# JustinMLu/legged_gym_custom

Measured on AMD Instinct MI355X. Metric: env-steps/sec (whole node), Go2 4096 envs, 1/2/4/8 MI355X, higher is better.
Workload: dtype f32; 1 GPU; go2, rsl_rl PPO/ROA iteration (24 env steps + 5x4 minibatch update); num_envs_per_gpu=4096, num_steps_per_env=24, global_envs=4096, parallelism=env-sharded dp1

## Files before the change

include/lgx.h:

```cpp
#ifndef LGX_H
#define LGX_H

#include <stdint.h>

#ifdef __cplusplus
extern "C" {
#endif

#define LGX_ABI_VERSION 13

#define LGX_MAX_DOF 12
#define LGX_MAX_LINKS 16
#define LGX_MAX_BODIES 24
#define LGX_MAX_FEET 4
#define LGX_MAX_PROPRIO 240
#define LGX_MAX_HEIGHT_POINTS 192
#define LGX_MAX_REWARDS 40
#define LGX_MAX_CANDIDATES 64
#define LGX_MAX_CONTACTS 16
#define LGX_MAX_PENALISED 24
#define LGX_MAX_TERMINATION 8
#define LGX_EVAL_METRICS 8
#define LGX_EVAL_CELL_COLS 12
#define LGX_MAX_ACTION_HISTORY 4
// ... 226 lines not shown
int64_t lgx_sizeof_task_params(void);
int64_t lgx_sizeof_buffers(void);

int lgx_create(const lgx_model* model, const lgx_task_params* params, int32_t device, lgx_env** out);
int lgx_bind(lgx_env* env, const lgx_buffers* buffers);
int lgx_step(lgx_env* env, uint64_t seed, uint64_t step_counter, void* hip_stream);
int lgx_step_dev(lgx_env* env, uint64_t seed, const uint64_t* d_step_counter, void* hip_stream);
int lgx_post_physics(lgx_env* env, uint64_t seed, uint64_t step_counter, void* hip_stream);
int lgx_physics(lgx_env* env, void* hip_stream);
int lgx_reset_envs(lgx_env* env, const uint8_t* env_mask, uint64_t seed, uint64_t reset_call, void* hip_stream);
int lgx_episode_extras(lgx_env* env, float* means, float* level_mean, uint8_t* time_outs, uint64_t* step_dev,
                       void* hip_stream);
int lgx_command_curriculum(lgx_env* env, uint64_t seed, uint64_t step_counter, const uint64_t* d_step_counter,
                           const double* global_sum_count, void* hip_stream);
int lgx_set_envs_per_wave(lgx_env* env, int32_t envs_per_wave);

typedef struct lgx_eval_buffers {
  float* acc;
  uint8_t* status;
  double* cells;
  uint32_t* overflow;
  int32_t cell_rows, cell_cols;
  const int32_t* cell_ids;
  float* push_rec;
  float settle_tol;
  double* push_cells;
  const int32_t* cmd_switch_step;
  float* cmd_rec;
  double* cmd_cells;
  float yaw_tol;
// ... 52 lines not shown
```

legged_gym_custom_amd/_abi.py:

```python
import ctypes as C

ABI_VERSION = 13
MAX_DOF = 12
MAX_LINKS = 16
MAX_BODIES = 24
MAX_FEET = 4
MAX_PROPRIO = 240
MAX_HEIGHT_POINTS = 192
MAX_REWARDS = 40
MAX_CANDIDATES = 64
MAX_CONTACTS = 16
MAX_PENALISED = 24
MAX_TERMINATION = 8
EVAL_METRICS = 8
EVAL_CELL_COLS = 12
MAX_ACTION_HISTORY = 4
EVAL_PUSH_REC = 4
EVAL_PUSH_COLS = 5
CMD_SEGMENTS = 4
EVAL_CMD_REC = 8
EVAL_CMD_COLS = 9
TRACE_COLS = 76
GAIT_FOOT_COLS = 16
GAIT_BODY_COLS = 12
# ... 167 lines not shown

u64, cint = C.c_uint64, C.c_int
SIGNATURES = {
    "lgx_abi_version": (i32, ()),
    **{name: (C.c_int64, ()) for name in SIZEOF},
    "lgx_create": (cint, (P, P, i32, C.POINTER(P))),
    "lgx_bind": (cint, (P, P)),
    "lgx_step": (cint, (P, u64, u64, P)),
    "lgx_step_dev": (cint, (P, u64, P, P)),
    "lgx_post_physics": (cint, (P, u64, u64, P)),
    "lgx_physics": (cint, (P, P)),
    "lgx_reset_envs": (cint, (P, P, u64, u64, P)),
    "lgx_episode_extras": (cint, (P, P, P, P, P, P)),
    "lgx_command_curriculum": (cint, (P, u64, u64, P, P, P)),
    "lgx_set_envs_per_wave": (cint, (P, i32)),
    "lgx_eval_begin": (cint, (P, P, P)),
    "lgx_eval_accumulate": (cint, (P, P, P)),
    "lgx_eval_reduce": (cint, (P, P, P)),
    "lgx_trace_begin": (cint, (P, P, P)),
    "lgx_trace_record": (cint, (P, P, P)),
    "lgx_trace_gather": (cint, (P, P, P, i32, P, P, P)),
    "lgx_gait_begin": (cint, (P, P, P)),
    "lgx_gait_record": (cint, (P, P, P)),
    "lgx_gait_reduce": (cint, (P, P, P)),
    "lgx_joint_begin": (cint, (P, P, P)),
    "lgx_joint_record": (cint, (P, P, P)),
    "lgx_joint_reduce": (cint, (P, P, P)),
    "lgx_last_error": (C.c_char_p, (P,)),
    "lgx_destroy": (None, (P,)),
}
# ... 12 lines not shown
```

legged_gym_custom_amd/_native.py:

```python
import ctypes as C
import os

from . import _abi, _cbind

LIB_PATH = os.environ.get("LGX_LIB") or os.path.join(os.path.dirname(os.path.abspath(__file__)), "lib", "liblgx.so")
_lib = None


class LgxError(RuntimeError):
    pass


def lib():
    global _lib
    if _lib is None:
        _lib = _cbind.load(LIB_PATH, "liblgx", _abi.SIGNATURES, _abi.STRUCTS, ("lgx_abi_version", _abi.ABI_VERSION),
                           _abi.SIZEOF, LgxError)
    return _lib


EXPORTED = list(_abi.SIGNATURES)


class NativeEnv:
# ... 20 lines not shown
            t = tensors.get(name)
            if t is None:
                setattr(self.buffers, name, None)
                continue
            if not t.is_contiguous():
                raise LgxError(f"buffer {name} must be contiguous")
            if t.device.type != self._dev_type:
                where = "host memory (device -1)" if self._dev_type == "cpu" else "the HIP device"
                raise LgxError(f"buffer {name} must live in {where} (got {t.device})")
            setattr(self.buffers, name, t.data_ptr())
            self._keep[name] = t
        self._check(self._L.lgx_bind(self.handle, C.byref(self.buffers)), "lgx_bind")

    def set_envs_per_wave(self, n):
        self._check(self._L.lgx_set_envs_per_wave(self.handle, int(n)), "lgx_set_envs_per_wave")

    def step(self, seed, step_counter, stream):
        self._check(self._L.lgx_step(self.handle, seed, step_counter, C.c_void_p(stream)), "lgx_step")

    def step_dev(self, seed, step_counter_tensor, stream):
        self._check(self._L.lgx_step_dev(self.handle, seed, C.c_void_p(step_counter_tensor.data_ptr()),
                                         C.c_void_p(stream)), "lgx_step_dev")

    def post_physics(self, seed, step_counter, stream):
        self._check(self._L.lgx_post_physics(self.handle, seed, step_counter, C.c_void_p(stream)), "lgx_post_physics")

    def reset_envs(self, mask, seed, call, stream):
        self._keep["_mask"] = mask
        self._check(self._L.lgx_reset_envs(self.handle, C.c_void_p(mask.data_ptr()), seed, call, C.c_void_p(stream)),
                    "lgx_reset_envs")
# ... 145 lines not shown
```

legged_gym_custom_amd/csrc/lgx_env.hip:

```cpp
#include <hip/hip_runtime.h>
#include "lgx_knobs.h"
#include <math.h>
#include <stddef.h>
#include <stdint.h>

#include "../../include/lgx.h"
#include "lgx_device.h"
#include "lgx_env_common.h"
#include "lgx_host.h"

namespace lgx {

constexpr int ASQ = 24;
constexpr int AMAX = 33;
constexpr int RW = 9;
constexpr int A_FLOATS = ASQ * ASQ > AMAX * (AMAX + 1) / 2 ? ASQ * ASQ : AMAX * (AMAX + 1) / 2;
constexpr int J9_FLOATS = MAXR * RW > A_FLOATS ? MAXR * RW : A_FLOATS;
constexpr int ROWS_FLOATS = MAXR * RW + J9_FLOATS;
extern __shared__ float lgx_dyn[];
struct DynTemps {
  float Fw[NL][3], Nw[NL][3];
  float Dl[4][6];
  float tot[16];
  float Sp[21];
};
static_assert(sizeof(DynTemps) <= ROWS_FLOATS * sizeof(float), "dynamics temporaries fit the arena");
LGX_DEV DynTemps& dtmp(float* A) { return *reinterpret_cast<DynTemps*>(A); }
LGX_DEV float* stg_U(float* A) { return A; }
LGX_DEV float* stg_cur(float* A, const lgx_task_params* Pm) { return A + 4 * rng_blocks(Pm); }
constexpr int HIST_LDS_MAX = 640;
__host__ __device__ inline bool hist_in_lds(const lgx_task_params* Pm) {
  return Pm->history_len * Pm->num_proprio <= HIST_LDS_MAX || Pm->num_proprio < 64;
}
LGX_DEV float* stg_hist(float* A, const lgx_task_params* Pm) { return stg_cur(A, Pm) + Pm->num_proprio; }
LGX_DEV float* stg_heights(float* A, const lgx_task_params* Pm) {
  return stg_hist(A, Pm) + (hist_in_lds(Pm) ? Pm->history_len * Pm->num_proprio : 0);
}
__host__ __device__ inline int64_t arena_floats(const lgx_task_params& p) {
  const int64_t post = 4 * (9 + (p.num_proprio + 3) / 4) + p.num_proprio +
                       (hist_in_lds(&p) ? (int64_t)p.history_len * p.num_proprio : 0) + p.num_height_points;
  return post > ROWS_FLOATS ? post : ROWS_FLOATS;
}

struct Sh {
  Scratch x;
  float root[13], cmd[4], fat[4], lch[4];
  int lc[4];
  float rterm[64];
  float jsum[16];
  long long ep_prev;
  int lc_prev[LGX_MAX_FEET];
  float lch_prev[LGX_MAX_FEET], fat_prev[LGX_MAX_FEET], jump_prev;
  float la_prev[NJ], lt_prev[NJ];
  float es[LGX_MAX_REWARDS + 4];
  float fric;
  long long ep;
  int reset, tout;
  int blew;
  float qb[4], pb[3], vo[3], wb[3];
// ... 27 lines not shown
  } while (0)
#else
#define PH(k) \
  do {        \
  } while (0)
#endif

#pragma clang fp contract(fast)

template <class T>
LGX_DEV const T* opaque(const T* p) {
  __asm__ volatile("" : "+s"(p));
  return p;
}

LGX_DEV int env_of_block(int b, int n) {
  const int q = n >> 3, r = n & 7, x = b & 7, j = b >> 3;
  return x * q + min(x, r) + j;
}

#ifndef LGX_ROW_PRIO
#define LGX_ROW_PRIO 9
#endif
#ifndef LGX_SLOT_PRIO
#define LGX_SLOT_PRIO 0
#endif

LGX_DEV int wave_slot() { return __builtin_amdgcn_s_getreg(4 | (3 << 11)) & 15; }
LGX_DEV void set_prio(int p) {
  if (p >= 3) __builtin_amdgcn_s_setprio(3);
// ... 171 lines not shown
    const float on = lane <= NJ ? 1.f : 0.f;
    const float rd[16] = {m, m * r.x, m * r.y, m * r.z,
                          Iw[0] + m * (rr - r.x * r.x), Iw[1] + m * (rr - r.y * r.y), Iw[2] + m * (rr - r.z * r.z),
                          Iw[3] - m * r.x * r.y, Iw[4] - m * r.x * r.z, Iw[5] - m * r.y * r.z,
                          F.x, F.y, F.z, Nt.x, Nt.y, Nt.z};
#pragma unroll
    for (int q = 0; q < 16; ++q) {
      float x = rd[q] * on;
      x += dpp_shr_t<0x111>(x);
      x += dpp_shr_t<0x112>(x);
      x += dpp_shr_t<0x114>(x);
      x += dpp_shr_t<0x118>(x);
      if (lane == 15) dtmp(A).tot[q] = x;
    }
  }
  __syncthreads();
}

struct DynOut {
  float hb[6];
  float hj;
  float xj[6];
  float dinv[3];
};

LGX_DEV void dynamics(Sh& s, float* A, int lane, DynOut& o) {
  const f3 p0 = ld3(s.P[0]);
  const float* tot = dtmp(A).tot;
  const int j = lane < NJ ? lane : NJ - 1, l = j / 3, a = j % 3;
  if (lane < NJ) {
    const int kj = 1 + j;
// ... 19 lines not shown
    const int q = lane - 8, lq = q / 6, e = q % 6;
    const int j1 = e < 3 ? e : (e == 5 ? 1 : 0);
    const int j2 = e < 3 ? e : (e == 3 ? 1 : 2);
    const int k1 = 1 + 3 * lq + j1, k2 = 1 + 3 * lq + j2;
    const f3 a1 = ld3(s.Ax[k1]), a2 = ld3(s.Ax[k2]), p1 = ld3(s.P[k1]), p2 = ld3(s.P[k2]);
    float acc = 0.f;
#pragma unroll
    for (int i = 0; i < 3; ++i) {
      if (i < j2) continue;
      const int k = 1 + 3 * lq + i;
      const f3 c = ld3(s.C[k]);
      acc += s.m[k] * dot(cross(a1, c - p1), cross(a2, c - p2)) + dot(a1, symv(s.I[k], a2));
    }
    dtmp(A).Dl[lq][e] = acc;
  }
  __syncthreads();
  float Di[6];
  sym3_inv(dtmp(A).Dl[l], Di);
#pragma unroll
  for (int c = 0; c < 3; ++c) o.dinv[c] = sym3(Di, a, c);
  if (lane < NJ && a == 0) {
#pragma unroll
    for (int q = 0; q < 6; ++q) s.Dinv[l][q] = Di[q];
  }
  float bj[6];
  {
    const float* B0 = s.Bc[3 * l];
    const float* B1 = s.Bc[3 * l + 1];
    const float* B2 = s.Bc[3 * l + 2];
#pragma unroll
    for (int r = 0; r < 6; ++r) {
      const float b0 = B0[r], b1 = B1[r], b2 = B2[r];
      o.xj[r] = o.dinv[0] * b0 + o.dinv[1] * b1 + o.dinv[2] * b2;
      bj[r] = a == 0 ? b0 : (a == 1 ? b1 : b2);
    }
  }
  if (lane < NJ) {
#pragma unroll
    for (int r = 0; r < 6; ++r) s.X[j][r] = o.xj[r];
  }
  __syncthreads();
  if (lane < 21) {
    const int q = lane;
    const int r = (q >= 1) + (q >= 3) + (q >= 6) + (q >= 10) + (q >= 15), c = q - r * (r + 1) / 2;
    float acc = 0.f;
#pragma unroll
    for (int jj = 0; jj < NJ; ++jj) acc += s.X[jj][r] * s.Bc[jj][c];
    dtmp(A).Sp[q] = acc;
  }
  __syncthreads();
  const float Mt = tot[0], Hx = tot[1], Hy = tot[2], Hz = tot[3];
  const float Ab[21] = {Mt, 0.f, Mt, 0.f, 0.f, Mt, 0.f, -Hz, Hy, tot[4], Hz, 0.f, -Hx, tot[7], tot[5],
                        -Hy, Hx, 0.f, tot[8], tot[9], tot[6]};
  float L[21];
#pragma unroll
  for (int q = 0; q < 21; ++q) L[q] = Ab[q] - dtmp(A).Sp[q];
  float inv[6];
#pragma unroll
  for (int c = 0; c < 6; ++c) {
    float d = L[pk(c, c)];
#pragma unroll
    for (int k = 0; k < c; ++k) d -= L[pk(c, k)] * L[pk(c, k)];
    const float lcc = sqrtf(fmaxf(d, 1e-12f));
    inv[c] = 1.0f / lcc;
#pragma unroll
// ... 75 lines not shown
  const int total_max = gmax<WL>(total);
  int* const T_end = reinterpret_cast<int*>(A);
  int* const T_ci = T_end + 64;
  int* const T_cj = T_end + 128;
  int* const T_i0 = T_end + 192;
  int* const T_j0 = T_end + 256;
  int* const T_w = T_end + 320;
  float* const T_p = A + 384;
  float* const R_ = A + 576;
  T_end[lane] = endp; T_ci[lane] = ci; T_cj[lane] = cj; T_i0[lane] = i0; T_j0[lane] = j0; T_w[lane] = w;
  T_p[lane] = p.x; T_p[64 + lane] = p.y; T_p[128 + lane] = p.z;
  float best = 3.0e38f, zs = -3.0e38f;
  f3 q = mk(0.f, 0.f, -3.0e38f), fn = mk(0.f, 0.f, 1.f);
  const int mystart = endp - cnt;
  for (int base = 0; base < total_max; base += WL) {
    __syncthreads();
    const int t = base + lane;
    float td2 = 3.0e38f, tz = -3.0e38f;
    f3 tq = mk(0.f, 0.f, -3.0e38f), tfn = mk(0.f, 0.f, 1.f);
    if (t < total) {
      int lo = 0, hi = WL - 1;
      while (lo < hi) {
        const int mid = (lo + hi) >> 1;
        if (T_end[mid] > t) hi = mid; else lo = mid + 1;
      }
      const int c = lo;
      const int k = t - (c ? T_end[c - 1] : 0);
      const int wc = T_w[c];
      const int i = T_i0[c] + k / wc, j = T_j0[c] + k % wc;
      const int cci = T_ci[c], ccj = T_cj[c];
      const f3 pc = mk(T_p[c], T_p[64 + c], T_p[128 + c]);
// ... 4 lines not shown
#pragma unroll
      for (int tri = 0; tri < 2; ++tri) {
        const f3 a = v00, b = tri == 0 ? v11 : v10, cc = tri == 0 ? v01 : v11;
        const f3 cpt = closest_on_triangle(pc, a, b, cc);
        const f3 dd = pc - cpt;
        const float d2 = dot(dd, dd);
        if (d2 < td2) { td2 = d2; tq = cpt; tfn = cross(b - a, cc - a); }
        float z;
        if (height_in_triangle(pc, a, b, cc, z)) tz = fmaxf(tz, z);
      }
    }
    R_[lane] = td2;
    R_[64 + lane] = tq.x; R_[128 + lane] = tq.y; R_[192 + lane] = tq.z;
    R_[256 + lane] = tfn.x; R_[320 + lane] = tfn.y; R_[384 + lane] = tfn.z;
    R_[448 + lane] = tz;
    __syncthreads();
    if (cnt > 0) {
      const int a0 = max(mystart, base) - base, a1 = min(endp, base + WL) - base;
      for (int sl = a0; sl < a1; ++sl) {
        const float d2 = R_[sl];
        if (d2 < best) {
          best = d2;
          q = mk(R_[64 + sl], R_[128 + sl], R_[192 + sl]);
          fn = mk(R_[256 + sl], R_[320 + sl], R_[384 + sl]);
        }
        zs = fmaxf(zs, R_[448 + sl]);
      }
    }
  }
  __syncthreads();
  TerrainHit h;
  if (best >= 3.0e38f) {
    h.depth = -3.0e38f;
    h.n = mk(0.f, 0.f, 1.f);
    return h;
  }
  const float dist = sqrtf(best);
  const bool below = p.z < zs;
  h.depth = below ? r + dist : r - dist;
  if (dist > 1e-6f) {
    h.n = (p - q) * ((below ? -1.0f : 1.0f) / dist);
  } else {
    h.n = fn * rsqrtf(fmaxf(dot(fn, fn), 1e-30f));
  }
  return h;
// ... 83 lines not shown
  }
  return a;
}

LGX_DEV float motor_strength(const lgx_task_params* Pm, const lgx_buffers& B, int e, int j) {
  return B.motor_strength ? B.motor_strength[(size_t)e * Pm->num_dof + j] : 1.0f;
}

LGX_DEV void sea_torques_lanes(Sh& s, float* A, const lgx_task_params* Pm_, const lgx_buffers& B, int e, int lane,
                               int sub) {
  const size_t NT = (size_t)Pm_->num_envs * Pm_->num_dof;
  const int u = lane & 7;
  {
    const float* src = &Pm_->sea_in_scale[0];
    for (int i = lane; i < SEA_WN; i += 64) A[i] = src[i];
    __syncthreads();
  }
#pragma unroll 1
  for (int pass = 0; pass < 2; ++pass) {
    const lgx_task_params* Pm = opaque(Pm_);
    int wb = 0;
    __asm__ volatile("" : "+s"(wb));
    const SeaW W{A + wb};
    const int j = pass * 8 + (lane >> 3);
    const bool on = j < NJ;
    const int jj = on ? j : NJ - 1;
    const size_t r = (size_t)e * Pm->num_dof + jj;
    float h0 = B.sea_hidden[r * 8 + u], c0 = B.sea_cell[r * 8 + u];
    float h1 = B.sea_hidden[(NT + r) * 8 + u], c1 = B.sea_cell[(NT + r) * 8 + u];
    const float in0 = (sea_action(s, Pm, B, e, jj, sub) * Pm->action_scale + Pm->default_dof_pos[jj]) - s.th[jj];
    const float x[2] = {in0 * Pm->sea_in_scale[0], s.thd[jj] * Pm->sea_in_scale[1]};
// ... 57 lines not shown
      g[2] = Di[4] * jlr[0] + Di[5] * jlr[1] + Di[2] * jlr[2];
    }
    float* zg = ZG + lane * RW;
    float arr = jlr[0] * g[0] + jlr[1] * g[1] + jlr[2] * g[2];
#pragma unroll
    for (int q = 0; q < 6; ++q) {
      const float* Si = s.Sinv[q];
      const float zq = Si[0] * yr[0] + Si[1] * yr[1] + Si[2] * yr[2] + Si[3] * yr[3] + Si[4] * yr[4] + Si[5] * yr[5];
      zg[q] = zq;
      arr += yr[q] * zq;
    }
    zg[6] = g[0]; zg[7] = g[1]; zg[8] = g[2];
    s.Arr[lane] = arr;
    s.lam[lane] = 0.f;
  }
  __syncthreads();
  PH(6);
  const int NRm = gmax<WL>(nrows);
  const bool tri = nrows > ASQ, stored = nrows <= AMAX;
  if (stored && row_lane) {
#pragma unroll 4
    for (int q = 0; q < NRm; ++q) {
      if (q < nrows) {
        const float* zg = ZG + q * RW;
        const float v = yr[0] * zg[0] + yr[1] * zg[1] + yr[2] * zg[2] + yr[3] * zg[3] + yr[4] * zg[4] + yr[5] * zg[5];
        const float vl = jlr[0] * zg[6] + jlr[1] * zg[7] + jlr[2] * zg[8];
        const float a = v + (s.rleg[q] == lr ? vl : 0.f);
        if (!tri) Am[q * nrows + lane] = a;
        else if (q >= lane) Am[q * (q + 1) / 2 + lane] = a;
      }
    }
  }
  __syncthreads();
  PH(7);
  {
    float w = w0, lam = 0.f;
    const float mu = s.mu;
    auto wave_shl1 = [](float v) {
      return __int_as_float(__builtin_amdgcn_update_dpp(0, __float_as_int(v), 0x130, 0xf, 0xf, false));
    };
    auto wave_shr1 = [](float v) {
      return __int_as_float(__builtin_amdgcn_update_dpp(0, __float_as_int(v), 0x138, 0xf, 0xf, false));
    };
    const float tg = row_lane ? s.tgt[lane] : 0.f;
    const float ia = row_lane ? 1.0f / s.Arr[lane] : 0.f;
    const int rlast = max(nrows - 3, 0);
    const int lc = max(min(lane, nrows - 1), 0);
    const int tl = lc * (lc + 1) / 2;
// ... 55 lines not shown
          const float d1 = gbcast<WL>(dl, ra_ + 1, rb_ + 1), d2 = gbcast<WL>(dl, ra_ + 2, rb_ + 2);
          lam = sel((unsigned)(lane - r - 1) < 2u && on, lam, lt);
          w += a1 * d1 + a2 * d2;
        }
      }
    };
    if constexpr (WL == 64) {
      if (!stored) sweeps(arow_otf);
      else if (tri) sweeps(arow_tri);
      else sweeps(arow_sq);
    } else {
      sweeps(arow_mix);
    }
    if (row_lane) s.lam[lane] = lam;
  }
  __syncthreads();
  PH(8);
}

template <bool TERRAIN, bool ACTNET, int WL>
LGX_DEV void substep(Sh& s, float* A, Sh* S0, float* A0, int astride, const lgx_model* M_,
                     const lgx_task_params* Pm_, const lgx_buffers& B, int lane_, int e, int sub, bool last) {
  const lgx_model* M = opaque(M_);
  const lgx_task_params* Pm = opaque(Pm_);
  const int lane = opaque_lane(lane_);
  const float dt = Pm->sim_dt;
  {
#pragma clang fp contract(off)
    if (ACTNET) {
      sea_torques_lanes(s, A, Pm, B, e, lane, sub);
    } else if (lane < NJ) {
// ... 14 lines not shown
      if (B.motor_strength) t = motor_strength(Pm, B, e, j) * t;
      s.tau[j] = fminf(fmaxf(t, -Pm->torque_limits[j]), Pm->torque_limits[j]);
    }
  }
  PH(1);
  kinematics<true>(s, A, M, Pm, lane);
  PH(2);
  DynOut dy;
  dynamics(s, A, lane, dy);
  const int jl_ = lane < NJ ? lane : NJ - 1, leg_ = jl_ / 3, pos_ = jl_ % 3;
  const float fj = lane < NJ ? s.tau[lane] - dy.hj : 0.f;
  if (lane < NJ) s.up[lane] = fj;
  float vb[6];
#pragma unroll
  for (int r = 0; r < 6; ++r) vb[r] = -dy.hb[r] - grow_sum16<WL>(dy.xj[r] * fj);
  __syncthreads();
  PH(3);
  {
    float zb[6];
#pragma unroll
    for (int r = 0; r < 6; ++r) {
      const float* Si = s.Sinv[r];
      zb[r] = Si[0] * vb[0] + Si[1] * vb[1] + Si[2] * vb[2] + Si[3] * vb[3] + Si[4] * vb[4] + Si[5] * vb[5];
    }
    if (lane < 6) {
      const float* Si = s.Sinv[lane];
      const float zl = Si[0] * vb[0] + Si[1] * vb[1] + Si[2] * vb[2] + Si[3] * vb[3] + Si[4] * vb[4] + Si[5] * vb[5];
      const float u0 = lane < 3 ? s.vo[lane] : s.wb[lane - 3];
      s.us[lane] = u0 + dt * zl;
    }
    if (lane < NJ) {
// ... 116 lines not shown
  const int nrows = nlim + 3 * ncon;
  const int nrw = gmax<WL>(nrows);
#if LGX_ROW_PRIO > 0
  {
    const int rp = nrw > LGX_ROW_PRIO * 3 ? 3 : nrw > LGX_ROW_PRIO * 2 ? 2 : nrw > LGX_ROW_PRIO ? 1 : 0;
    set_prio(LGX_SLOT_PRIO ? max(rp, min(wave_slot(), 3)) : rp);
  }
#endif
  if (lane == 0) { s.nrows = nrows; s.nlim = nlim; s.ncon = ncon; }
#ifdef LGX_PHASE_CLOCK
  if (lane == 0) {
    s.phacc[16] = max(s.phacc[16], (uint32_t)nrows);
    s.phacc[17] += nrows > AMAX ? 1u : 0u;
  }
#endif
  __syncthreads();
  PH(5);
  if constexpr (WL == 64) {
    solve_rows<64>(s, A, Pm, lane, nrows, nlim, ncon);
  } else if (nrw <= WL) {
    solve_rows<WL>(s, A, Pm, lane, nrows, nlim, ncon);
  } else {
    const int wl = (int)__lane_id();
#pragma unroll 1
    for (int g = 0; g < 64 / WL; ++g) {
      Sh& sg = S0[g];
      const int nr = gval<WL>(nrows, g), nli = gval<WL>(nlim, g), nco = gval<WL>(ncon, g);
      solve_rows<64>(sg, A0 + (size_t)g * astride, Pm, wl, nr, nli, nco);
    }
  }
  {
// ... 12 lines not shown
    }
    if (lane < 6) {
      float zl = 0.f;
#pragma unroll
      for (int q = 0; q < 6; ++q) zl = lane == q ? Z[q] : zl;
      s.up[lane] = s.us[lane] + zl;
    }
    if (lane < NJ) {
      const float* Xj = s.X[lane];
      float v = s.us[6 + lane] + G;
#pragma unroll
      for (int q = 0; q < 6; ++q) v -= Xj[q] * Z[q];
      s.up[6 + lane] = v;
    }
  }
  __syncthreads();
  PH(9);
  if (last && lane < LGX_MAX_BODIES) {
    float f[3] = {0.f, 0.f, 0.f};
    const int ncm = gmax<WL>(ncon);
    for (int c = 0; c < ncm; ++c) {
      if (c >= ncon || s.cbody[c] != lane) continue;
      const int r = nlim + 3 * c;
      if constexpr (!TERRAIN) {
        f[2] += s.lam[r]; f[0] += s.lam[r + 1]; f[1] += s.lam[r + 2];
      } else {
        f3 t1, t2;
        const f3 n = ld3(s.cn[c]);
        contact_tangents(n, t1, t2);
        const f3 fc = n * s.lam[r] + t1 * s.lam[r + 1] + t2 * s.lam[r + 2];
        f[0] += fc.x; f[1] += fc.y; f[2] += fc.z;
// ... 18 lines not shown
    float qn[4];
    qn[3] = dq[3] * q[3] - (dq[0] * q[0] + dq[1] * q[1] + dq[2] * q[2]);
    qn[0] = dq[3] * q[0] + q[3] * dq[0] + (dq[1] * q[2] - dq[2] * q[1]);
    qn[1] = dq[3] * q[1] + q[3] * dq[1] + (dq[2] * q[0] - dq[0] * q[2]);
    qn[2] = dq[3] * q[2] + q[3] * dq[2] + (dq[0] * q[1] - dq[1] * q[0]);
    float nq = rsqrtf(qn[0] * qn[0] + qn[1] * qn[1] + qn[2] * qn[2] + qn[3] * qn[3]);
#pragma unroll
    for (int i = 0; i < 4; ++i) s.qb[i] = qn[i] * nq;
    st3(s.vo, v);
    st3(s.wb, w);
  }
  if (lane < NJ) {
    s.thd[lane] = s.up[6 + lane];
    s.th[lane] += dt * s.thd[lane];
  }
  __syncthreads();
  PH(10);
}

#pragma clang fp contract(off)


template <int WL>
LGX_DEV void reset_env(const lgx_task_params* Pm, const lgx_buffers& B, Sh& s, float* A, int e, int lane,
                       bool after_init, bool zero_carried, bool sums_in_lds) {
  const int D = Pm->num_dof;
  const float* U = stg_U(A);
  if (lane == 0) reset_env_head(Pm, B, s, U, e, after_init);
  if (lane < D) {
    s.th[lane] = Pm->default_dof_pos[lane] + rand_range(0.0f, 0.9f, U[S_DOF + lane]);
    s.thd[lane] = 0.0f;
// ... 17 lines not shown
  }
  if (Pm->task_kind == LGX_TASK_GO2 && lane < Pm->num_feet) {
    if (B.feet_air_time) B.feet_air_time[e * Pm->num_feet + lane] = 0.f;
    B.last_contacts[e * Pm->num_feet + lane] = 0;
    B.last_contact_heights[e * Pm->num_feet + lane] = 0.f;
  }
  const int K = Pm->num_reward_terms + (Pm->has_termination_reward ? 1 : 0);
  for (int k = lane; k < K; k += WL) {
    float* es = B.episode_sums + (size_t)e * K + k;
    const float sum = sums_in_lds ? s.es[k] : *es;
    if (B.episode_stats) atomicAdd(B.episode_stats + k, sum);
    if (sums_in_lds && B.curriculum_vals && k == Pm->curriculum_term) B.curriculum_vals[e] = sum;
    *es = 0.f;
  }
  if (lane == 0 && B.episode_stats) atomicAdd(B.episode_stats + K, 1.0f);
  __syncthreads();
}

template <int WL>
LGX_DEV void fill_uniforms(float* A, uint64_t seed, uint32_t gid, uint64_t step, uint32_t stream, int lane, int nblk) {
  for (int b = lane; b < nblk; b += WL) {
    uint32_t o[4];
    philox4x32_10(gid, (uint32_t)step, (uint32_t)b | (stream << 16), (uint32_t)(step >> 32), (uint32_t)seed,
                  (uint32_t)(seed >> 32), o);
    float* U = stg_U(A);
    U[4 * b + 0] = u01(o[0]); U[4 * b + 1] = u01(o[1]);
    U[4 * b + 2] = u01(o[2]); U[4 * b + 3] = u01(o[3]);
  }
  __syncthreads();
}

LGX_DEV void joint_sums(const lgx_task_params* Pm, const lgx_buffers& B, Sh& s, float* A, int e, int lane) {
  const int D = Pm->num_dof;
  const int j = lane < D ? lane : 0;
  const float on = lane < D ? 1.0f : 0.0f;
  const float la = s.la_prev[j], lt = s.lt_prev[j];
  const float q = s.th[j], qd = s.thd[j], tau = s.tau[j], q0 = Pm->default_dof_pos[j];
  const float dq = q - q0;
  float v[J_N];
  v[J_ACTION_RATE] = sq(la - s.act[j]);
  v[J_DELTA_TORQUES] = sq(tau - lt);
  v[J_DOF_ACC] = sq((s.ldv[j] - qd) / Pm->dt);
  v[J_DOF_ERROR] = sq(dq);
  {
// ... 54 lines not shown
    long ix = (long)(px / Pm->horizontal_scale), iy = (long)(py / Pm->horizontal_scale);
    ix = ix < 0 ? 0 : (ix > Pm->hf_rows - 2 ? Pm->hf_rows - 2 : ix);
    iy = iy < 0 ? 0 : (iy > Pm->hf_cols - 2 ? Pm->hf_cols - 2 : iy);
    int16_t h1 = B.height_samples[ix * Pm->hf_cols + iy];
    int16_t h2 = B.height_samples[(ix + 1) * Pm->hf_cols + iy];
    int16_t h3 = B.height_samples[ix * Pm->hf_cols + iy + 1];
    int16_t h = h1 < h2 ? h1 : h2;
    h = h < h3 ? h : h3;
    stg_heights(A, Pm)[i] = (float)h * Pm->vertical_scale;
  }
}

#ifndef LGX_SEA_WAVES
#define LGX_SEA_WAVES 4
#endif
template <bool PHYSICS, bool TERRAIN, bool ACTNET, int EPW>
__global__ __launch_bounds__(64, ACTNET ? LGX_SEA_WAVES : (EPW == 2 ? 2 : 4)) void env_step_kernel(const lgx_model* __restrict__ M,
                                                      const lgx_task_params* __restrict__ Pm,
                                                      const lgx_buffers* __restrict__ Bp, uint64_t seed,
                                                      uint64_t step_arg, const uint64_t* __restrict__ step_dev) {
  constexpr int WL = 64 / EPW;
  __shared__ Sh S_[EPW];
  const int grp = grp_of_lane<WL>();
  Sh& s = S_[grp];
  const int astride = (int)arena_floats(*Pm);
  float* const AR = lgx_dyn + (EPW == 1 ? 0 : grp * astride);
  const lgx_buffers& B = *Bp;
  const uint64_t step = step_dev ? *step_dev : step_arg;
  const int e = EPW * env_of_block(blockIdx.x, gridDim.x) + grp;
  const int lane = EPW == 1 ? (int)threadIdx.x : (int)(threadIdx.x & (WL - 1));
#if LGX_SLOT_PRIO
  set_prio(min(wave_slot(), 3));
#endif
  const int D = Pm->num_dof, A = Pm->num_actions, NB = Pm->num_bodies;
  const uint32_t gid = (uint32_t)(Pm->env_id_offset + e);

  float* root_g = B.root_states + (size_t)e * 13;
  if (lane < A) {
    float a = B.actions_in[(size_t)e * A + lane];
    a = clipf(a, -Pm->clip_actions, Pm->clip_actions);
    s.act[lane] = a;
    B.actions[(size_t)e * A + lane] = a;
  }
  if (lane < D) {
    s.th[lane] = B.dof_state[((size_t)e * D + lane) * 2];
// ... 18 lines not shown
  if (lane < A) s.la_prev[lane] = B.last_actions[(size_t)e * A + lane];
  if (lane < D) s.lt_prev[lane] = B.last_torques[(size_t)e * D + lane];
  {
    const int KS0 = Pm->num_reward_terms + (Pm->has_termination_reward ? 1 : 0);
    for (int k = lane; k < KS0; k += WL) s.es[k] = B.episode_sums[(size_t)e * KS0 + k];
  }
  if (Pm->task_kind == LGX_TASK_GO2 && lane < Pm->num_feet) {
    s.lc_prev[lane] = B.last_contacts[e * Pm->num_feet + lane];
    s.lch_prev[lane] = B.last_contact_heights[e * Pm->num_feet + lane];
    s.fat_prev[lane] = B.feet_air_time ? B.feet_air_time[e * Pm->num_feet + lane] : 0.f;
  }
#ifdef LGX_PHASE_CLOCK
  if (lane < 20) s.phacc[lane] = 0u;
  if (lane == 0) s.phlast = clock64();
#endif
  __syncthreads();

  if (PHYSICS) {
    if (lane == 0) {
      float q[4] = {s.root[3], s.root[4], s.root[5], s.root[6]};
      float n = rsqrtf(q[0] * q[0] + q[1] * q[1] + q[2] * q[2] + q[3] * q[3]);
      for (int i = 0; i < 4; ++i) s.qb[i] = q[i] * n;
      for (int i = 0; i < 3; ++i) { s.pb[i] = s.root[i]; s.wb[i] = s.root[10 + i]; }
      float R[9];
      quat_to_R(s.qb, R);
      f3 rc = mv(R, mk(M->link_com[0][0] + s.cadd[0], M->link_com[0][1] + s.cadd[1], M->link_com[0][2] + s.cadd[2]));
      f3 vo = ld3(s.root + 7) - cross(ld3(s.wb), rc);
      st3(s.vo, vo);
    }
    __syncthreads();
    PH(0);
    for (int sub = 0; sub < Pm->decimation; ++sub) {
      if (!ACTNET && B.action_delay) {
        stage_actuator_action(s, Pm, B, e, lane, sub);
        __syncthreads();
      }
      substep<TERRAIN, ACTNET, WL>(s, AR, S_, lgx_dyn, astride, M, Pm, B, lane, e, sub, sub == Pm->decimation - 1);
    }
    if (!ACTNET && B.action_delay) {
      const int ln = opaque_lane(lane), A = opaque(Pm)->num_actions;
      if (ln < A) s.act[ln] = B.actions[(size_t)e * A + ln];
    }
    __syncthreads();
    {
      bool bad = false;
      if (lane < D) bad = !(isfinite(s.th[lane]) && isfinite(s.thd[lane]) && isfinite(s.tau[lane]));
      if (lane < A) bad = bad || !isfinite(s.act[lane]);
      if (lane < 3) bad = bad || !(isfinite(s.pb[lane]) && isfinite(s.vo[lane]) && isfinite(s.wb[lane]));
      if (lane < 4) bad = bad || !isfinite(s.qb[lane]);
      if (lane < NB) bad = bad || !(isfinite(s.cf[lane][0]) && isfinite(s.cf[lane][1]) && isfinite(s.cf[lane][2]));
      if (gballot<WL>(bad) != 0ull) {
        if (lane < D) { s.th[lane] = Pm->default_dof_pos[lane]; s.thd[lane] = 0.f; s.tau[lane] = 0.f; }
        if (lane < A) { s.act[lane] = 0.f; B.actions[(size_t)e * A + lane] = 0.f; }
        if (lane < 3) { s.pb[lane] = isfinite(s.root[lane]) ? s.root[lane] : 0.f; s.vo[lane] = 0.f; s.wb[lane] = 0.f; }
        if (lane < 4) s.qb[lane] = lane == 3 ? 1.f : 0.f;
        if (lane < NB) { s.cf[lane][0] = 0.f; s.cf[lane][1] = 0.f; s.cf[lane][2] = 0.f; }
        if (lane == 0) {
          s.blew = 1;
          if (B.blowup_count) atomicAdd(B.blowup_count, 1u);
        }
      }
      __syncthreads();
    }
    kinematics<false>(s, AR, M, Pm, lane);
    float root[13];
    {
      float R[9];
      quat_to_R(s.qb, R);
      f3 rc = mv(R, mk(M->link_com[0][0] + s.cadd[0], M->link_com[0][1] + s.cadd[1], M->link_com[0][2] + s.cadd[2]));
      f3 vc = ld3(s.vo) + cross(ld3(s.wb), rc);
      root[0] = s.pb[0]; root[1] = s.pb[1]; root[2] = s.pb[2];
      root[3] = s.qb[0]; root[4] = s.qb[1]; root[5] = s.qb[2]; root[6] = s.qb[3];
      root[7] = vc.x; root[8] = vc.y; root[9] = vc.z;
      root[10] = s.wb[0]; root[11] = s.wb[1]; root[12] = s.wb[2];
    }
    __syncthreads();
    if (lane < 13) s.root[lane] = root[lane];
    if (lane < NB) {
      const int k = M->body_link[lane];
      f3 off = ld3(M->body_offset[lane]);
      f3 o = mv(s.R[k], off);
      f3 pos = ld3(s.P[k]) + o;
      bool primary = off.x == 0.f && off.y == 0.f && off.z == 0.f;
      f3 lv = ld3(s.V[k]) + cross(ld3(s.W[k]), primary ? (ld3(s.C[k]) - ld3(s.P[k])) : o);
      float Rb[9];
      mm(s.R[k], M->body_rot[lane], Rb);
      float tr = Rb[0] + Rb[4] + Rb[8], qq[4];
      if (tr > 0.f) {
        float sc = sqrtf(tr + 1.f) * 2.f;
        qq[3] = 0.25f * sc; qq[0] = (Rb[7] - Rb[5]) / sc; qq[1] = (Rb[2] - Rb[6]) / sc; qq[2] = (Rb[3] - Rb[1]) / sc;
      } else if (Rb[0] > Rb[4] && Rb[0] > Rb[8]) {
// ... 6 lines not shown
        float sc = sqrtf(1.f + Rb[8] - Rb[0] - Rb[4]) * 2.f;
        qq[3] = (Rb[3] - Rb[1]) / sc; qq[0] = (Rb[2] + Rb[6]) / sc; qq[1] = (Rb[5] + Rb[7]) / sc; qq[2] = 0.25f * sc;
      }
      if (qq[3] < 0.f) for (int i = 0; i < 4; ++i) qq[i] = -qq[i];
      float* rb = B.rigid_body_states + ((size_t)e * NB + lane) * 13;
      rb[0] = pos.x; rb[1] = pos.y; rb[2] = pos.z;
      rb[3] = qq[0]; rb[4] = qq[1]; rb[5] = qq[2]; rb[6] = qq[3];
      rb[7] = lv.x; rb[8] = lv.y; rb[9] = lv.z;
      const float* w = s.W[k];
      rb[10] = w[0]; rb[11] = w[1]; rb[12] = w[2];
      s.rbz[lane] = pos.z;
      float* cfo = B.contact_forces + ((size_t)e * NB + lane) * 3;
      cfo[0] = s.cf[lane][0]; cfo[1] = s.cf[lane][1]; cfo[2] = s.cf[lane][2];
    }
    if (lane < D) B.torques[(size_t)e * D + lane] = s.tau[lane];
    __syncthreads();
    PH(11);
  } else {
    if (lane < NB) {
      const float* cfi = B.contact_forces + ((size_t)e * NB + lane) * 3;
      s.cf[lane][0] = cfi[0]; s.cf[lane][1] = cfi[1]; s.cf[lane][2] = cfi[2];
      s.rbz[lane] = B.rigid_body_states[((size_t)e * NB + lane) * 13 + 2];
    }
    if (lane < D) s.tau[lane] = B.torques[(size_t)e * D + lane];
    __syncthreads();
  }

  constexpr int HV = 320 / WL;
  float hv[HV];
  {
    const int HPn = Pm->history_len * Pm->num_proprio;
    const float* hsrc = B.obs_history + (size_t)e * HPn;
#pragma unroll
    for (int t = 0; t < HV; ++t) {
      const int i = lane + WL * t;
      hv[t] = i < HPn ? hsrc[i] : 0.f;
    }
  }
  fill_uniforms<WL>(AR, seed, gid, step, 0, lane, rng_blocks(Pm));
  PH(12);
// ... 51 lines not shown
    if (B.push_step && (long long)B.push_step[e] == ep) scheduled_push(root, B.push_dvel + (size_t)e * 3);
    int reset = 0;
    for (int i = 0; i < Pm->n_termination; ++i) {
      const float* c = s.cf[Pm->termination_idx[i]];
      reset |= nrm3(c[0], c[1], c[2]) > 1.0f;
    }
    int tout = ep > Pm->max_episode_length && !s.blew;
    reset |= tout;
    reset |= x.pg[2] > 0.0f;
    if (Pm->parkour) reset |= root[2] < -1.0f;
    reset |= s.blew;
    s.reset = reset;
    s.tout = tout;
    x.jump = s.jump_prev;
  }
  __syncthreads();
  PH(13);
  get_heights<WL>(Pm, B, s, AR, lane);
  __syncthreads();
  joint_sums(Pm, B, s, AR, e, lane);
  __syncthreads();
  const int K = Pm->num_reward_terms;
  const int KS = K + (Pm->has_termination_reward ? 1 : 0);
  for (int k = lane; k < K; k += WL)
    s.rterm[k] = s.blew ? 0.0f : reward_term(Pm, s, Pm->reward_ids[k]) * Pm->reward_scales[k];
  __syncthreads();
  const int reset = s.reset;
  if (lane == 0) {
    float rew = 0.0f;
    for (int k = 0; k < K; ++k) rew += s.rterm[k];
    if (Pm->only_positive_rewards) rew = rew < 0.0f ? 0.0f : rew;
    if (Pm->has_termination_reward) {
      float v = (float)(reset && !s.tout && !s.blew) * Pm->termination_scale;
      rew += v;
      s.rterm[K] = v;
    }
    B.rew[e] = rew;
    B.reset[e] = (uint8_t)reset;
    B.time_out[e] = (uint8_t)s.tout;
    if (B.blew_up) B.blew_up[e] = (uint8_t)s.blew;
  }
  __syncthreads();
  for (int k = lane; k < KS; k += WL) {
    const float v = s.es[k] + s.rterm[k];
    s.es[k] = v;
    B.episode_sums[(size_t)e * KS + k] = v;
  }
  __syncthreads();
  PH(14);
  if (reset) reset_env<WL>(Pm, B, s, AR, e, lane, true, false, true);

  const int Pp = Pm->num_proprio, H = Pm->history_len;
  const Scratch& x = s.x;
  if (go2 && Pm->parkour && lane == 0) {
    int outl = 0;
    for (int i = 0; i < Pm->num_height_points; ++i) outl += fabsf(stg_heights(AR, Pm)[i]) > 0.1f;
    s.x.jump = (float)(outl >= 8);
  }
  for (int i = lane; i < Pp; i += WL) {
    float v;
    if (go2) {
      if (i < 3) v = x.bav[i] * Pm->obs_scale_ang_vel;
      else if (i == 3) v = x.roll;
// ... 25 lines not shown
  float* const hist = stg_hist(AR, Pm);
  const float* const cur = stg_cur(AR, Pm);
  const bool hl = hist_in_lds(Pm);
  const long long ep = s.ep;
  const float co = Pm->clip_obs;
  float* obs = B.obs + (size_t)e * Pm->num_obs;
  float* cr = B.critic ? B.critic + (size_t)e * Pm->num_critic : nullptr;
  if (hl) {
#pragma unroll
    for (int t = 0; t < HV; ++t) {
      const int i = lane + WL * t;
      if (i < H * Pp) hist[i] = reset ? 0.f : hv[t];
    }
    for (int i = lane + WL * HV; i < H * Pp; i += WL) hist[i] = reset ? 0.f : hist_g[i];
  }
  __syncthreads();
  if (hl) {
    for (int i = lane; i < H * Pp; i += WL) {
      float v = clipf(hist[i], -co, co);
      obs[i] = v;
      if (go2 && cr) cr[i] = v;
    }
  } else {
    const int HP = H * Pp, HP1 = (H - 1) * Pp;
#pragma unroll
    for (int t = 0; t < (MAXHIST + WL - 1) / WL; ++t) {
      const int i = lane + WL * t;
      if (WL * t >= HP) break;
      if (i < HP) {
        const float old = reset ? 0.f : (t < HV ? hv[t < HV ? t : 0] : hist_g[i]);
        const float v = clipf(old, -co, co);
// ... 59 lines not shown
  if (lane < 4) B.commands[e * 4 + lane] = s.cmd[lane];
  if (go2 && lane < Pm->num_feet && !reset) {
    B.last_contacts[e * Pm->num_feet + lane] = (uint8_t)s.lc[lane];
    B.last_contact_heights[e * Pm->num_feet + lane] = s.lch[lane];
    if (B.feet_air_time) B.feet_air_time[e * Pm->num_feet + lane] = s.fat[lane];
  }
  if (lane == 0) B.episode_length[e] = ep;
  if (B.rpy_phase && lane < 8) {
    float v = lane == 0 ? x.roll : lane == 1 ? x.pitch : lane == 2 ? x.yaw : lane < 7 ? x.ph[lane - 3] : x.jump;
    B.rpy_phase[e * 8 + lane] = v;
  }
  if (B.measured_heights)
    for (int i = lane; i < Pm->num_height_points; i += WL)
      B.measured_heights[(size_t)e * Pm->num_height_points + i] = stg_heights(AR, Pm)[i];
#ifdef LGX_PHASE_CLOCK
  __syncthreads();
  PH(15);
  __syncthreads();
  if (lane == 0) {
    s.phacc[18] = __builtin_amdgcn_s_getreg(4 | (31 << 11));
    s.phacc[19] = __builtin_amdgcn_s_getreg(20 | (31 << 11));
  }
  __syncthreads();
  if (g_phase_out && lane < NPH) g_phase_out[(size_t)e * NPH + lane] = s.phacc[lane];
#endif
}

__global__ __launch_bounds__(64) void reset_kernel(const lgx_task_params* __restrict__ Pm,
                                                   const lgx_buffers* __restrict__ Bp,
                                                   const uint8_t* __restrict__ mask, uint64_t seed, uint64_t call) {
  __shared__ Sh s;
  const lgx_buffers& B = *Bp;
  const int e = blockIdx.x;
  const int lane = threadIdx.x;
  if (!mask[e]) return;
  const int D = Pm->num_dof;
  fill_uniforms<64>(lgx_dyn, seed, (uint32_t)(Pm->env_id_offset + e), call, 1, lane, rng_blocks(Pm));
  if (lane < 13) s.root[lane] = B.root_states[(size_t)e * 13 + lane];
// ... 2 lines not shown
  reset_env<64>(Pm, B, s, lgx_dyn, e, lane, true, true, false);
  if (lane < 13) B.root_states[(size_t)e * 13 + lane] = s.root[lane];
  if (lane < D) {
    B.dof_state[((size_t)e * D + lane) * 2] = s.th[lane];
    B.dof_state[((size_t)e * D + lane) * 2 + 1] = s.thd[lane];
  }
  if (lane < 4) B.commands[e * 4 + lane] = s.cmd[lane];
  if (lane == 0) { B.episode_length[e] = s.ep; B.reset[e] = 1; }
}

}

#include <stdio.h>

#include <initializer_list>
#include <string>

struct lgx_env {
  lgx_model model;
  lgx_task_params params;
  lgx_buffers buffers;
  lgx_model* d_model = nullptr;
  lgx_task_params* d_params = nullptr;
  lgx_buffers* d_buffers = nullptr;
  int device = 0;
  bool host = false;
  bool bound = false;
  bool stats_clean = false;
  int epw = 0;
  std::string err;
};

static int fail(lgx_env* env, const std::string& msg) {
  if (env) env->err = msg;
  return -1;
}

#define HIP_OK(call)                                                                   \
  do {                                                                                 \
    hipError_t _e = (call);                                                            \
    if (_e != hipSuccess) return fail(env, std::string(#call ": ") + hipGetErrorString(_e)); \
  } while (0)

extern "C" {
// ... 129 lines not shown
    HIP_OK(hipMemsetAsync(env->buffers.episode_stats, 0, sizeof(float) * (KS + 1), st));
  env->stats_clean = false;
  const bool terrain = env->params.mesh_type != LGX_MESH_PLANE, actnet = env->params.actuator_net != 0;
  static const int epw_env = [] {
    const char* v = LGX_DEV_KNOB("LGX_ENVS_PER_WAVE");
    return v && atoi(v) == 1 ? 1 : 2;
  }();
  const int want = env->epw ? env->epw : (terrain ? 1 : epw_env);
  const int epw = (!actnet && N % 2 == 0 && want == 2) ? 2 : 1;
  auto kern = epw == 2 ? (!physics ? lgx::env_step_kernel<false, false, false, 2>
                                   : (terrain ? lgx::env_step_kernel<true, true, false, 2>
                                              : lgx::env_step_kernel<true, false, false, 2>))
            : !physics ? lgx::env_step_kernel<false, false, false, 1>
            : actnet   ? (terrain ? lgx::env_step_kernel<true, true, true, 1> : lgx::env_step_kernel<true, false, true, 1>)
                       : (terrain ? lgx::env_step_kernel<true, true, false, 1> : lgx::env_step_kernel<true, false, false, 1>);
  const size_t dyn = sizeof(float) * (size_t)lgx::arena_floats(env->params) * epw;
  hipLaunchKernelGGL(kern, dim3(N / epw), dim3(64), dyn, st, env->d_model, env->d_params, env->d_buffers, seed, step,
                     step_dev);
  HIP_OK(hipGetLastError());
  return 0;
}

int lgx_set_envs_per_wave(lgx_env* env, int32_t envs_per_wave) {
  if (!env) return -2;
  if (envs_per_wave < 0 || envs_per_wave > 2) return fail(env, "lgx_set_envs_per_wave: 0, 1 or 2");
  env->epw = envs_per_wave;
  return 0;
}

int lgx_step(lgx_env* env, uint64_t seed, uint64_t step_counter, void* hip_stream) {
  return launch_step(env, seed, step_counter, nullptr, hip_stream, true);
}

int lgx_step_dev(lgx_env* env, uint64_t seed, const uint64_t* d_step_counter, void* hip_stream) {
// ... 966 lines not shown
```

Baseline: 4.950 million env-steps/s.

## Pack several env wavefronts per workgroup and use wave-local barriers

The step kernel now launches blocks of several 64-lane wavefronts, by default four for plane terrain and one for terrain or actuator-net. Each wave handles its own env unit, with its per-env state (Sh) moved from static into 16-byte-aligned dynamic LDS. Every __syncthreads becomes a wavefront-scoped fence plus wave barrier, so waves in the same block never wait on each other. The aim is to cut workgroup count and dispatch overhead and raise residency. The trade-off is that launch bounds now declare 256 threads with the same min-occupancy value, which tightens the register budget and could cause spills.

```diff
diff --git a/include/lgx.h b/include/lgx.h
--- a/include/lgx.h
+++ b/include/lgx.h
@@ -7,7 +7,7 @@
 extern "C" {
 #endif
 
-#define LGX_ABI_VERSION 13
+#define LGX_ABI_VERSION 14
 
 #define LGX_MAX_DOF 12
 #define LGX_MAX_LINKS 16
@@ -264,6 +264,7 @@
 int lgx_command_curriculum(lgx_env* env, uint64_t seed, uint64_t step_counter, const uint64_t* d_step_counter,
                            const double* global_sum_count, void* hip_stream);
 int lgx_set_envs_per_wave(lgx_env* env, int32_t envs_per_wave);
+int lgx_set_waves_per_block(lgx_env* env, int32_t waves_per_block);
 
 typedef struct lgx_eval_buffers {
   float* acc;
diff --git a/legged_gym_custom_amd/_abi.py b/legged_gym_custom_amd/_abi.py
--- a/legged_gym_custom_amd/_abi.py
+++ b/legged_gym_custom_amd/_abi.py
@@ -1,6 +1,6 @@
 import ctypes as C
 
-ABI_VERSION = 13
+ABI_VERSION = 14
 MAX_DOF = 12
 MAX_LINKS = 16
 MAX_BODIES = 24
@@ -205,6 +205,7 @@
     "lgx_episode_extras": (cint, (P, P, P, P, P, P)),
     "lgx_command_curriculum": (cint, (P, u64, u64, P, P, P)),
     "lgx_set_envs_per_wave": (cint, (P, i32)),
+    "lgx_set_waves_per_block": (cint, (P, i32)),
     "lgx_eval_begin": (cint, (P, P, P)),
     "lgx_eval_accumulate": (cint, (P, P, P)),
     "lgx_eval_reduce": (cint, (P, P, P)),
diff --git a/legged_gym_custom_amd/_native.py b/legged_gym_custom_amd/_native.py
--- a/legged_gym_custom_amd/_native.py
+++ b/legged_gym_custom_amd/_native.py
@@ -58,6 +58,9 @@
 
     def set_envs_per_wave(self, n):
         self._check(self._L.lgx_set_envs_per_wave(self.handle, int(n)), "lgx_set_envs_per_wave")
+
+    def set_waves_per_block(self, n):
+        self._check(self._L.lgx_set_waves_per_block(self.handle, int(n)), "lgx_set_waves_per_block")
 
     def step(self, seed, step_counter, stream):
         self._check(self._L.lgx_step(self.handle, seed, step_counter, C.c_void_p(stream)), "lgx_step")
diff --git a/legged_gym_custom_amd/csrc/lgx_env.hip b/legged_gym_custom_amd/csrc/lgx_env.hip
--- a/legged_gym_custom_amd/csrc/lgx_env.hip
+++ b/legged_gym_custom_amd/csrc/lgx_env.hip
@@ -17,7 +17,8 @@
 constexpr int A_FLOATS = ASQ * ASQ > AMAX * (AMAX + 1) / 2 ? ASQ * ASQ : AMAX * (AMAX + 1) / 2;
 constexpr int J9_FLOATS = MAXR * RW > A_FLOATS ? MAXR * RW : A_FLOATS;
 constexpr int ROWS_FLOATS = MAXR * RW + J9_FLOATS;
-extern __shared__ float lgx_dyn[];
+extern __shared__ __align__(16) float lgx_dyn[];
+extern __shared__ __align__(16) float lgx_sh_dyn[];
 struct DynTemps {
   float Fw[NL][3], Nw[NL][3];
   float Dl[4][6];
@@ -39,10 +40,10 @@
 __host__ __device__ inline int64_t arena_floats(const lgx_task_params& p) {
   const int64_t post = 4 * (9 + (p.num_proprio + 3) / 4) + p.num_proprio +
                        (hist_in_lds(&p) ? (int64_t)p.history_len * p.num_proprio : 0) + p.num_height_points;
-  return post > ROWS_FLOATS ? post : ROWS_FLOATS;
-}
-
-struct Sh {
+  return ((post > ROWS_FLOATS ? post : ROWS_FLOATS) + 3) & ~(int64_t)3;
+}
+
+struct alignas(16) Sh {
   Scratch x;
   float root[13], cmd[4], fat[4], lch[4];
   int lc[4];
@@ -100,6 +101,12 @@
   return p;
 }
 
+LGX_DEV void wave_sync() {
+  __builtin_amdgcn_fence(__ATOMIC_RELEASE, "wavefront");
+  __builtin_amdgcn_wave_barrier();
+  __builtin_amdgcn_fence(__ATOMIC_ACQUIRE, "wavefront");
+}
+
 LGX_DEV int env_of_block(int b, int n) {
   const int q = n >> 3, r = n & 7, x = b & 7, j = b >> 3;
   return x * q + min(x, r) + j;
@@ -301,7 +308,7 @@
       if (lane == 15) dtmp(A).tot[q] = x;
     }
   }
-  __syncthreads();
+  wave_sync();
 }
 
 struct DynOut {
@@ -351,7 +358,7 @@
     }
     dtmp(A).Dl[lq][e] = acc;
   }
-  __syncthreads();
+  wave_sync();
   float Di[6];
   sym3_inv(dtmp(A).Dl[l], Di);
 #pragma unroll
@@ -376,7 +383,7 @@
 #pragma unroll
     for (int r = 0; r < 6; ++r) s.X[j][r] = o.xj[r];
   }
-  __syncthreads();
+  wave_sync();
   if (lane < 21) {
     const int q = lane;
     const int r = (q >= 1) + (q >= 3) + (q >= 6) + (q >= 10) + (q >= 15), c = q - r * (r + 1) / 2;
@@ -385,7 +392,7 @@
     for (int jj = 0; jj < NJ; ++jj) acc += s.X[jj][r] * s.Bc[jj][c];
     dtmp(A).Sp[q] = acc;
   }
-  __syncthreads();
+  wave_sync();
   const float Mt = tot[0], Hx = tot[1], Hy = tot[2], Hz = tot[3];
   const float Ab[21] = {Mt, 0.f, Mt, 0.f, 0.f, Mt, 0.f, -Hz, Hy, tot[4], Hz, 0.f, -Hx, tot[7], tot[5],
                         -Hy, Hx, 0.f, tot[8], tot[9], tot[6]};
@@ -491,7 +498,7 @@
   f3 q = mk(0.f, 0.f, -3.0e38f), fn = mk(0.f, 0.f, 1.f);
   const int mystart = endp - cnt;
   for (int base = 0; base < total_max; base += WL) {
-    __syncthreads();
+    wave_sync();
     const int t = base + lane;
     float td2 = 3.0e38f, tz = -3.0e38f;
     f3 tq = mk(0.f, 0.f, -3.0e38f), tfn = mk(0.f, 0.f, 1.f);
@@ -526,7 +533,7 @@
     R_[64 + lane] = tq.x; R_[128 + lane] = tq.y; R_[192 + lane] = tq.z;
     R_[256 + lane] = tfn.x; R_[320 + lane] = tfn.y; R_[384 + lane] = tfn.z;
     R_[448 + lane] = tz;
-    __syncthreads();
+    wave_sync();
     if (cnt > 0) {
       const int a0 = max(mystart, base) - base, a1 = min(endp, base + WL) - base;
       for (int sl = a0; sl < a1; ++sl) {
@@ -540,7 +547,7 @@
       }
     }
   }
-  __syncthreads();
+  wave_sync();
   TerrainHit h;
   if (best >= 3.0e38f) {
     h.depth = -3.0e38f;
@@ -654,7 +661,7 @@
   {
     const float* src = &Pm_->sea_in_scale[0];
     for (int i = lane; i < SEA_WN; i += 64) A[i] = src[i];
-    __syncthreads();
+    wave_sync();
   }
 #pragma unroll 1
   for (int pass = 0; pass < 2; ++pass) {
@@ -742,7 +749,7 @@
     s.Arr[lane] = arr;
     s.lam[lane] = 0.f;
   }
-  __syncthreads();
+  wave_sync();
   PH(6);
   const int NRm = gmax<WL>(nrows);
   const bool tri = nrows > ASQ, stored = nrows <= AMAX;
@@ -759,7 +766,7 @@
       }
     }
   }
-  __syncthreads();
+  wave_sync();
   PH(7);
   {
     float w = w0, lam = 0.f;
@@ -845,7 +852,7 @@
     }
     if (row_lane) s.lam[lane] = lam;
   }
-  __syncthreads();
+  wave_sync();
   PH(8);
 }
 
@@ -890,7 +897,7 @@
   float vb[6];
 #pragma unroll
   for (int r = 0; r < 6; ++r) vb[r] = -dy.hb[r] - grow_sum16<WL>(dy.xj[r] * fj);
-  __syncthreads();
+  wave_sync();
   PH(3);
   {
     float zb[6];
@@ -1037,7 +1044,7 @@
     s.phacc[17] += nrows > AMAX ? 1u : 0u;
   }
 #endif
-  __syncthreads();
+  wave_sync();
   PH(5);
   if constexpr (WL == 64) {
     solve_rows<64>(s, A, Pm, lane, nrows, nlim, ncon);
@@ -1080,7 +1087,7 @@
       s.up[6 + lane] = v;
     }
   }
-  __syncthreads();
+  wave_sync();
   PH(9);
   if (last && lane < LGX_MAX_BODIES) {
     float f[3] = {0.f, 0.f, 0.f};
@@ -1129,7 +1136,7 @@
     s.thd[lane] = s.up[6 + lane];
     s.th[lane] += dt * s.thd[lane];
   }
-  __syncthreads();
+  wave_sync();
   PH(10);
 }
 
@@ -1177,7 +1184,7 @@
     *es = 0.f;
   }
   if (lane == 0 && B.episode_stats) atomicAdd(B.episode_stats + K, 1.0f);
-  __syncthreads();
+  wave_sync();
 }
 
 template <int WL>
@@ -1190,7 +1197,7 @@
     U[4 * b + 0] = u01(o[0]); U[4 * b + 1] = u01(o[1]);
     U[4 * b + 2] = u01(o[2]); U[4 * b + 3] = u01(o[3]);
   }
-  __syncthreads();
+  wave_sync();
 }
 
 LGX_DEV void joint_sums(const lgx_task_params* Pm, const lgx_buffers& B, Sh& s, float* A, int e, int lane) {
@@ -1275,21 +1282,40 @@
 #ifndef LGX_SEA_WAVES
 #define LGX_SEA_WAVES 4
 #endif
+#ifndef LGX_WPB_PLANE
+#define LGX_WPB_PLANE 4
+#endif
+#ifndef LGX_WPB_TERRAIN
+#define LGX_WPB_TERRAIN 1
+#endif
+#ifndef LGX_WPB_SEA
+#define LGX_WPB_SEA 1
+#endif
+__host__ __device__ inline int64_t wave_lds_floats(const lgx_task_params& p, int epw) {
+  return (int64_t)epw * ((int64_t)(sizeof(Sh) / sizeof(float)) + arena_floats(p));
+}
+static_assert(sizeof(Sh) % 16 == 0 && alignof(Sh) == 16, "Sh images tile the dynamic LDS in 16-B units");
 template <bool PHYSICS, bool TERRAIN, bool ACTNET, int EPW>
-__global__ __launch_bounds__(64, ACTNET ? LGX_SEA_WAVES : (EPW == 2 ? 2 : 4)) void env_step_kernel(const lgx_model* __restrict__ M,
+__global__ __launch_bounds__(256, ACTNET ? LGX_SEA_WAVES : (EPW == 2 ? 2 : 4)) void env_step_kernel(const lgx_model* __restrict__ M,
                                                       const lgx_task_params* __restrict__ Pm,
                                                       const lgx_buffers* __restrict__ Bp, uint64_t seed,
-                                                      uint64_t step_arg, const uint64_t* __restrict__ step_dev) {
+                                                      uint64_t step_arg, const uint64_t* __restrict__ step_dev,
+                                                      int units) {
   constexpr int WL = 64 / EPW;
-  __shared__ Sh S_[EPW];
+  const int wpb = (int)(blockDim.x >> 6);
+  const int wv = __builtin_amdgcn_readfirstlane((int)(threadIdx.x >> 6));
+  const int unit = env_of_block(blockIdx.x, gridDim.x) * wpb + wv;
+  if (unit >= units) return;
   const int grp = grp_of_lane<WL>();
+  const int astride = (int)arena_floats(*Pm);
+  Sh* const S_ = reinterpret_cast<Sh*>(lgx_sh_dyn) + wv * EPW;
   Sh& s = S_[grp];
-  const int astride = (int)arena_floats(*Pm);
-  float* const AR = lgx_dyn + (EPW == 1 ? 0 : grp * astride);
+  float* const AR0 = lgx_dyn + (wpb * EPW) * (int)(sizeof(Sh) / sizeof(float)) + (wv * EPW) * astride;
+  float* const AR = AR0 + (EPW == 1 ? 0 : grp * astride);
   const lgx_buffers& B = *Bp;
   const uint64_t step = step_dev ? *step_dev : step_arg;
-  const int e = EPW * env_of_block(blockIdx.x, gridDim.x) + grp;
-  const int lane = EPW == 1 ? (int)threadIdx.x : (int)(threadIdx.x & (WL - 1));
+  const int e = EPW * unit + grp;
+  const int lane = (int)(threadIdx.x & (WL - 1));
 #if LGX_SLOT_PRIO
   set_prio(min(wave_slot(), 3));
 #endif
@@ -1338,7 +1364,7 @@
   if (lane < 20) s.phacc[lane] = 0u;
   if (lane == 0) s.phlast = clock64();
 #endif
-  __syncthreads();
+  wave_sync();
 
   if (PHYSICS) {
     if (lane == 0) {
@@ -1352,20 +1378,20 @@
       f3 vo = ld3(s.root + 7) - cross(ld3(s.wb), rc);
       st3(s.vo, vo);
     }
-    __syncthreads();
+    wave_sync();
     PH(0);
     for (int sub = 0; sub < Pm->decimation; ++sub) {
       if (!ACTNET && B.action_delay) {
         stage_actuator_action(s, Pm, B, e, lane, sub);
-        __syncthreads();
+        wave_sync();
       }
-      substep<TERRAIN, ACTNET, WL>(s, AR, S_, lgx_dyn, astride, M, Pm, B, lane, e, sub, sub == Pm->decimation - 1);
+      substep<TERRAIN, ACTNET, WL>(s, AR, S_, AR0, astride, M, Pm, B, lane, e, sub, sub == Pm->decimation - 1);
     }
     if (!ACTNET && B.action_delay) {
       const int ln = opaque_lane(lane), A = opaque(Pm)->num_actions;
       if (ln < A) s.act[ln] = B.actions[(size_t)e * A + ln];
     }
-    __syncthreads();
+    wave_sync();
     {
       bool bad = false;
       if (lane < D) bad = !(isfinite(s.th[lane]) && isfinite(s.thd[lane]) && isfinite(s.tau[lane]));
@@ -1384,7 +1410,7 @@
           if (B.blowup_count) atomicAdd(B.blowup_count, 1u);
         }
       }
-      __syncthreads();
+      wave_sync();
     }
     kinematics<false>(s, AR, M, Pm, lane);
     float root[13];
@@ -1398,7 +1424,7 @@
       root[7] = vc.x; root[8] = vc.y; root[9] = vc.z;
       root[10] = s.wb[0]; root[11] = s.wb[1]; root[12] = s.wb[2];
     }
-    __syncthreads();
+    wave_sync();
     if (lane < 13) s.root[lane] = root[lane];
     if (lane < NB) {
       const int k = M->body_link[lane];
@@ -1435,7 +1461,7 @@
       cfo[0] = s.cf[lane][0]; cfo[1] = s.cf[lane][1]; cfo[2] = s.cf[lane][2];
     }
     if (lane < D) B.torques[(size_t)e * D + lane] = s.tau[lane];
-    __syncthreads();
+    wave_sync();
     PH(11);
   } else {
     if (lane < NB) {
@@ -1444,7 +1470,7 @@
       s.rbz[lane] = B.rigid_body_states[((size_t)e * NB + lane) * 13 + 2];
     }
     if (lane < D) s.tau[lane] = B.torques[(size_t)e * D + lane];
-    __syncthreads();
+    wave_sync();
   }
 
   constexpr int HV = 320 / WL;
@@ -1526,17 +1552,17 @@
     s.tout = tout;
     x.jump = s.jump_prev;
   }
-  __syncthreads();
+  wave_sync();
   PH(13);
   get_heights<WL>(Pm, B, s, AR, lane);
-  __syncthreads();
+  wave_sync();
   joint_sums(Pm, B, s, AR, e, lane);
-  __syncthreads();
+  wave_sync();
   const int K = Pm->num_reward_terms;
   const int KS = K + (Pm->has_termination_reward ? 1 : 0);
   for (int k = lane; k < K; k += WL)
     s.rterm[k] = s.blew ? 0.0f : reward_term(Pm, s, Pm->reward_ids[k]) * Pm->reward_scales[k];
-  __syncthreads();
+  wave_sync();
   const int reset = s.reset;
   if (lane == 0) {
     float rew = 0.0f;
@@ -1552,13 +1578,13 @@
     B.time_out[e] = (uint8_t)s.tout;
     if (B.blew_up) B.blew_up[e] = (uint8_t)s.blew;
   }
-  __syncthreads();
+  wave_sync();
   for (int k = lane; k < KS; k += WL) {
     const float v = s.es[k] + s.rterm[k];
     s.es[k] = v;
     B.episode_sums[(size_t)e * KS + k] = v;
   }
-  __syncthreads();
+  wave_sync();
   PH(14);
   if (reset) reset_env<WL>(Pm, B, s, AR, e, lane, true, false, true);
 
@@ -1614,7 +1640,7 @@
     }
     for (int i = lane + WL * HV; i < H * Pp; i += WL) hist[i] = reset ? 0.f : hist_g[i];
   }
-  __syncthreads();
+  wave_sync();
   if (hl) {
     for (int i = lane; i < H * Pp; i += WL) {
       float v = clipf(hist[i], -co, co);
@@ -1704,14 +1730,14 @@
     for (int i = lane; i < Pm->num_height_points; i += WL)
       B.measured_heights[(size_t)e * Pm->num_height_points + i] = stg_heights(AR, Pm)[i];
 #ifdef LGX_PHASE_CLOCK
-  __syncthreads();
+  wave_sync();
   PH(15);
-  __syncthreads();
+  wave_sync();
   if (lane == 0) {
     s.phacc[18] = __builtin_amdgcn_s_getreg(4 | (31 << 11));
     s.phacc[19] = __builtin_amdgcn_s_getreg(20 | (31 << 11));
   }
-  __syncthreads();
+  wave_sync();
   if (g_phase_out && lane < NPH) g_phase_out[(size_t)e * NPH + lane] = s.phacc[lane];
 #endif
 }
@@ -1744,6 +1770,7 @@
 #include <stdio.h>
 
 #include <initializer_list>
+#include <map>
 #include <string>
 
 struct lgx_env {
@@ -1758,6 +1785,8 @@
   bool bound = false;
   bool stats_clean = false;
   int epw = 0;
+  int wpb = 0;
+  std::map<const void*, size_t> dyn_allowed;
   std::string err;
 };
 
@@ -1917,10 +1946,27 @@
             : !physics ? lgx::env_step_kernel<false, false, false, 1>
             : actnet   ? (terrain ? lgx::env_step_kernel<true, true, true, 1> : lgx::env_step_kernel<true, false, true, 1>)
                        : (terrain ? lgx::env_step_kernel<true, true, false, 1> : lgx::env_step_kernel<true, false, false, 1>);
-  const size_t dyn = sizeof(float) * (size_t)lgx::arena_floats(env->params) * epw;
-  hipLaunchKernelGGL(kern, dim3(N / epw), dim3(64), dyn, st, env->d_model, env->d_params, env->d_buffers, seed, step,
-                     step_dev);
+  const int wpb = env->wpb ? env->wpb : (actnet ? LGX_WPB_SEA : terrain ? LGX_WPB_TERRAIN : LGX_WPB_PLANE);
+  const int units = N / epw;
+  const size_t dyn = sizeof(float) * (size_t)lgx::wave_lds_floats(env->params, epw) * wpb;
+  if (dyn > 64 * 1024) {
+    size_t& allowed = env->dyn_allowed[(const void*)kern];
+    if (dyn > allowed) {
+      HIP_OK(hipFuncSetAttribute((const void*)kern, hipFuncAttributeMaxDynamicSharedMemorySize, (int)dyn));
+      allowed = dyn;
+    }
+  }
+  hipLaunchKernelGGL(kern, dim3((units + wpb - 1) / wpb), dim3(64 * wpb), dyn, st, env->d_model, env->d_params,
+                     env->d_buffers, seed, step, step_dev, units);
   HIP_OK(hipGetLastError());
+  return 0;
+}
+
+int lgx_set_waves_per_block(lgx_env* env, int32_t waves_per_block) {
+  if (!env) return -2;
+  if (waves_per_block != 0 && waves_per_block != 1 && waves_per_block != 4)
+    return fail(env, "lgx_set_waves_per_block: 0, 1 or 4");
+  env->wpb = waves_per_block;
   return 0;
 }
 
```

Result: no change. 4.964 million env-steps/s, median of 6 (+0.3%).
